# rogerhh/gaussian-splatting-lm

Measured on AMD Instinct MI355X. Metric: CG matvecs/sec + raster Mpix/s, 1M Gaussians @1080p, 1/2/4/8 GPU, higher is better.
Workload: dtype f32; 1 GPU; LM CG iteration, 1000000 Gaussians SH3, 1x1920x1080 view(s) per GPU (BASELINE configs[2]; configs[3] at 8 GPUs); P=1000000, sh_degree=3, width=1920, height=1080, views_total=1, parallelism=views sharded x1, exchange=none, sh_rest_projected=True

## Files before the change

### gaussian-splatting-lm_amd/csrc/api.hip

```cpp
#include <cstring>
#include <string>
#include <vector>
#include "gslm_kernels.hpp"

namespace gslm {

static thread_local std::string g_last_error;
void set_error(const std::string& msg) { g_last_error = msg; }

thread_local DebugSync g_debug;

int launch_failed(hipError_t e, const char* file, int line) {
  const char* base = std::strrchr(file, '/');
  set_error(std::string(g_debug.on ? "kernel failed (debug mode: stream synchronised after the launch at " : "kernel launch (") +
            (base ? base + 1 : file) + ":" + std::to_string(line) + "): " + hipGetErrorString(e));
  return GSLM_ERR_HIP;
}

namespace {

struct Carver {
  char* base;
  size_t off = 0;
  template <typename T>
// ... 1031 lines not shown
}

size_t gslm_active_union_bytes(int64_t P) { return active_work_layout(P, nullptr, nullptr, nullptr, nullptr); }

int gslm_active_union(const gslm_view_ws* ws, int32_t nviews, int64_t P, void* work, size_t work_bytes, int32_t* ids_dev,
                      uint32_t* hrow_dev, uint32_t* aflags_dev, int64_t* count_dev, void* stream) {
  if (!ws || nviews < 1 || P < 0 || P > MAX_P || !work || !count_dev || !hrow_dev || (P > 0 && (!ids_dev || !aflags_dev))) {
    set_error("active_union: NULL argument, nviews below 1 or P out of range");
    return GSLM_ERR_INVALID;
  }
  for (int b = 0; b < nviews; ++b)
    if (ws[b].num_rendered < 0 || (ws[b].num_rendered > 0 && P > 0 && (!ws[b].geom || !ws[b].scratch))) {
      set_error("active_union: negative num_rendered or a NULL workspace of a view that rendered");
      return GSLM_ERR_INVALID;
    }
  if (work_bytes < gslm_active_union_bytes(P)) {
    set_error("active_union: work area below gslm_active_union_bytes(P)");
    return GSLM_ERR_CAPACITY;
  }
  for (int b = 0; b < nviews; ++b)
    if (ws[b].num_rendered > 0 && ws[b].scratch_bytes < gslm_scratch_bytes(P, ws[b].num_rendered)) {
      set_error("active_union: scratch workspace too small");
      return GSLM_ERR_CAPACITY;
    }
  std::vector<GeomBufs> gbs(nviews);
  std::vector<ScratchBufs> sbs(nviews);
  std::vector<int64_t> nr(nviews);
  for (int b = 0; b < nviews; ++b) {
    nr[b] = ws[b].num_rendered;
    if (nr[b] == 0) continue;
    geom_layout(P, const_cast<void*>(ws[b].geom), &gbs[b]);
    scratch_layout(P, nr[b], const_cast<void*>(ws[b].scratch), &sbs[b]);
  }
  uint32_t *flags, *tmp, *total;
  active_work_layout(P, work, &flags, &tmp, &total);
  return launch_active_union(gbs.data(), sbs.data(), nr.data(), nviews, P, flags, tmp, total, ids_dev, hrow_dev,
                             aflags_dev, count_dev, (hipStream_t)stream);
}

int gslm_inspect_rowmap(const void* geom, int64_t P, int64_t N, const void* scratch, size_t scratch_bytes,
                        uint32_t* goff, uint32_t* hscan, void* stream) {
  if (P < 0 || N < 0 || !geom || !scratch) { set_error("inspect_rowmap: NULL workspace or negative size"); return GSLM_ERR_INVALID; }
  if (scratch_bytes < gslm_scratch_bytes(P, N)) { set_error("inspect_rowmap: scratch workspace too small"); return GSLM_ERR_CAPACITY; }
  GeomBufs gb;
  ScratchBufs sb;
  geom_layout(P, const_cast<void*>(geom), &gb);
  scratch_layout(P, N, const_cast<void*>(scratch), &sb);
  hipStream_t s = (hipStream_t)stream;
  if (goff && P > 0) GSLM_HIP_CHECK(hipMemcpyAsync(goff, gb.goff, (size_t)P * 4, hipMemcpyDeviceToDevice, s));
  if (hscan) GSLM_HIP_CHECK(hipMemcpyAsync(hscan, sb.hscan, (size_t)(N + 1) * 4, hipMemcpyDeviceToDevice, s));
  return GSLM_OK;
}

int gslm_active_pack(const float* src, float* dst, const int32_t* active_ids, int64_t n_active, int64_t P,
                     const int32_t* widths, int32_t ngroups, int64_t tail_n, void* stream) {
  return launch_active_pack(true, src, dst, active_ids, n_active, P, widths, ngroups, tail_n, (hipStream_t)stream);
}

int gslm_active_unpack(const float* src, float* dst, const int32_t* active_ids, int64_t n_active, int64_t P,
                       const int32_t* widths, int32_t ngroups, int64_t tail_n, void* stream) {
  return launch_active_pack(false, src, dst, active_ids, n_active, P, widths, ngroups, tail_n, (hipStream_t)stream);
}

int gslm_sh_rest_project(const gslm_view* view, const gslm_gaussians* gi, int32_t mode, const float* in,
                         int64_t in_stride, float* out, int64_t out_stride, void* stream) {
  ViewK v;
  GaussK g;
  int st;
  if (!view || !gi) { set_error("sh_rest_project: NULL view / gaussians"); return GSLM_ERR_INVALID; }
  if ((st = make_view(view, gi->max_coeffs, &v))) return st;
  if ((st = make_gauss(gi, &v, &g, false))) return st;
  if (mode != 0 && mode != 1) { set_error("sh_rest_project: mode must be 0 (expand) or 1 (project)"); return GSLM_ERR_INVALID; }
  if (g.P > 0 && g.M > 1 && (!in || !out || !g.means3D)) { set_error("sh_rest_project: NULL buffer"); return GSLM_ERR_INVALID; }
  const int64_t full = 3 * (int64_t)(g.M - 1);
  if ((mode == 0 && (in_stride < 3 || out_stride < full)) || (mode == 1 && (in_stride < full || out_stride < 3))) {
    set_error("sh_rest_project: strides too small for [P,3] / [P,M-1,3] rows");
    return GSLM_ERR_INVALID;
  }
  return launch_sh_rest_project(v, g, mode, in, in_stride, out, out_stride, (hipStream_t)stream);
}

static int rest_views(const char* who, const gslm_view* views, int32_t nviews, const gslm_gaussians* gi, ViewK* vk,
                      GaussK* g) {
  if (!views || !gi || nviews < 1 || nviews > GSLM_MAX_REST_VIEWS) {
    set_error(std::string(who) + ": NULL views / gaussians or nviews outside 1..GSLM_MAX_REST_VIEWS");
    return GSLM_ERR_INVALID;
  }
  int st;
  for (int b = 0; b < nviews; ++b) {
    if ((st = make_view(&views[b], gi->max_coeffs, &vk[b]))) return st;
    if (vk[b].D != vk[0].D) {
      set_error(std::string(who) + ": the views must share one SH degree");
      return GSLM_ERR_INVALID;
    }
  }
  if ((st = make_gauss(gi, &vk[0], g, false))) return st;
  if (g->P > 0 && !g->means3D) {
    set_error(std::string(who) + ": NULL means3D");
    return GSLM_ERR_INVALID;
  }
  return GSLM_OK;
}

int gslm_rest_basis(const gslm_view* views, int32_t nviews, const gslm_gaussians* gi, float* R_out, void* stream) {
  ViewK vk[GSLM_MAX_REST_VIEWS];
  GaussK g;
// ... 247 lines not shown
```

### gaussian-splatting-lm_amd/csrc/forward.hip

```cpp
#include "gslm_internal.hpp"
#include "gslm_kernels.hpp"

namespace gslm {

template <bool RAW, bool STAGE>
__global__ __launch_bounds__(256) void k_preprocess(ViewK v, GaussK g, float4* __restrict__ rec,
                                                     uint32_t* __restrict__ depth_key,
                                                     uint32_t* __restrict__ tiles, uint2* __restrict__ rect,
                                                     uint32_t* __restrict__ clampw, int* __restrict__ radii_out,
                                                     int lead) {
  extern __shared__ __attribute__((aligned(16))) float s_sh[];
  const int64_t i = (int64_t)blockIdx.x * blockDim.x + threadIdx.x;
  if (STAGE) {
    const int64_t i0 = (int64_t)blockIdx.x * blockDim.x;
    const int64_t nv = min((int64_t)blockDim.x, g.P - i0);
    const int64_t total = nv * g.rest_stride;
    const float* rows = g.rest - lead + i0 * g.rest_stride;
    const float4* src4 = reinterpret_cast<const float4*>(rows);
    float4* dst4 = reinterpret_cast<float4*>(s_sh);
    for (int64_t e = threadIdx.x; e < total / 4; e += blockDim.x) dst4[e] = src4[e];
    for (int64_t e = (total / 4) * 4 + threadIdx.x; e < total; e += blockDim.x) s_sh[e] = rows[e];
    __syncthreads();
    g.rest = s_sh + lead;
    g.rest_base = i0;
  }
  if (i >= g.P) return;
  tiles[i] = 0u;
  depth_key[i] = 0xFFFFFFFFu;
  if (radii_out) radii_out[i] = 0;
  PreOut o;
  o.depth = 0.f;
  const bool vis = preprocess_one<RAW>(v, g, i, o);
  if (o.depth > 0.2f) depth_key[i] = __float_as_uint(o.depth);
  if (!vis) return;

  const float4 r0 = make_float4(o.x, o.y, o.conic[0], o.conic[1]);
  const float4 r1 = make_float4(o.conic[2], o.opac, o.rgb[0], o.rgb[1]);
  const float4 r2 = make_float4(o.rgb[2], 1.0f / o.depth, __uint_as_float(o.clamped), o.tq);
  rec[RECS * i + 0] = r0;
  rec[RECS * i + 1] = r1;
  rec[RECS * i + 2] = r2;
  tiles[i] = (uint32_t)((o.rmax_x - o.rmin_x) * (o.rmax_y - o.rmin_y));
  const uint2 rc = make_uint2((uint32_t)o.rmin_x | ((uint32_t)o.rmin_y << 16), (uint32_t)o.rmax_x | ((uint32_t)o.rmax_y << 16));
  rect[i] = rc;
  rec[RECS * i + 3] = make_float4(__uint_as_float(rc.x), __uint_as_float(rc.y), 0.f, 0.f);
  clampw[i] = o.clamped;
  if (radii_out) radii_out[i] = o.radius;
}

__device__ __forceinline__ void glds16(const float4* src, float4* lds_dst) {
  __builtin_amdgcn_global_load_lds((const __attribute__((address_space(1))) void*)src,
                                   (__attribute__((address_space(3))) void*)lds_dst, 16, 0, 0);
}

// ... 389 lines not shown
}

__global__ __launch_bounds__(256) void k_tile_neff(ViewK v, const uint32_t* __restrict__ n_contrib,
                                                    uint32_t* __restrict__ neff) {
  const int tile = blockIdx.x, tile_x = tile % v.gx, tile_y = tile / v.gx;
  int px, py;
  tile_pixel(tile_x, tile_y, threadIdx.x, px, py);
  int wm = (px < v.W && py < v.H) ? (int)n_contrib[(int64_t)py * v.W + px] : 0;
#pragma unroll
  for (int o = 32; o >= 1; o >>= 1) wm = max(wm, __shfl_xor(wm, o));
  if ((threadIdx.x & 63) == 0) neff[4 * tile + (threadIdx.x >> 6)] = (uint32_t)wm;
}

__global__ __launch_bounds__(256) void k_tile_cost(const uint2* __restrict__ ranges,
                                                    const uint32_t* __restrict__ point_list,
                                                    const uint32_t* __restrict__ neff, uint32_t* __restrict__ cost) {
  __shared__ uint32_t s_c[4][4];
  const int tile = blockIdx.x, tid = threadIdx.x, w = tid >> 6;
  const uint2 r = ranges[tile];
  const uint32_t len = r.y - r.x;
  uint32_t wm[4];
#pragma unroll
  for (int q = 0; q < 4; ++q) wm[q] = min(neff[4 * tile + q], len);
  const int n_eff = (int)max(max(wm[0], wm[1]), max(wm[2], wm[3]));
  uint32_t tot[4] = {0u, 0u, 0u, 0u}, vjp = 0u;
  for (int base = 0; base < n_eff; base += 256) {
    const int pos = n_eff - 1 - (base + tid);
    uint32_t m = 0u;
    if (pos >= 0) {
      const uint32_t e = point_list[r.x + pos];
      m = pl_mask(e) & (((uint32_t)pos < wm[0] ? 1u : 0u) | ((uint32_t)pos < wm[1] ? 2u : 0u) |
                        ((uint32_t)pos < wm[2] ? 4u : 0u) | ((uint32_t)pos < wm[3] ? 8u : 0u));
    }
#pragma unroll
    for (int q = 0; q < 4; ++q) {
      const uint32_t c = (uint32_t)__popcll(__ballot((m >> q) & 1u));
      if ((tid & 63) == 0) s_c[w][q] = c;
    }
    __syncthreads();
    uint32_t b0 = 0u, b1 = 0u;
#pragma unroll
    for (int q = 0; q < 4; ++q) {
      const uint32_t c0 = s_c[0][q] + s_c[1][q], c1 = s_c[2][q] + s_c[3][q];
      tot[q] += c0 + c1;
      b0 = max(b0, c0);
      b1 = max(b1, c1);
    }
    vjp += b0 + b1;
    __syncthreads();
  }
  if (tid == 0) cost[tile] = max(max(tot[0], tot[1]), max(tot[2], tot[3])) + vjp;
}

__device__ __forceinline__ uint32_t eff_mask(uint32_t e, uint32_t pos, const uint32_t* wm4) {
  const uint32_t wb = (pos < wm4[0] ? 1u : 0u) | (pos < wm4[1] ? 2u : 0u) | (pos < wm4[2] ? 4u : 0u) |
                      (pos < wm4[3] ? 8u : 0u);
  return pl_mask(e) & wb;
}

__global__ __launch_bounds__(256) void k_row_flags(int64_t N, int gx, const uint32_t* __restrict__ keys,
                                                    const uint32_t* __restrict__ point_list,
                                                    const uint2* __restrict__ ranges, const uint32_t* __restrict__ neff,
                                                    const uint32_t* __restrict__ goff, const uint2* __restrict__ rect,
                                                    uint32_t* __restrict__ slots, uint32_t* __restrict__ flags) {
  const int64_t k = (int64_t)blockIdx.x * blockDim.x + threadIdx.x;
  if (k >= N) return;
  const uint32_t t = keys[k];
  const uint32_t e = point_list[k];
  const uint32_t g = pl_id(e);
  const uint32_t o = row_slot(goff[g], rect[g], (int)(t % (uint32_t)gx), (int)(t / (uint32_t)gx));
  slots[k] = o;
  flags[o] = eff_mask(e, (uint32_t)k - ranges[t].x, neff + 4 * (size_t)t) ? 1u : 0u;
}

__global__ __launch_bounds__(256) void k_row_final(int64_t N, const uint32_t* __restrict__ hscan,
                                                    uint32_t* __restrict__ slots) {
  const int64_t k = (int64_t)blockIdx.x * blockDim.x + threadIdx.x;
  if (k < N) slots[k] = hscan[slots[k]];
}

int launch_lm_rowmap(const ViewK& v, const GeomBufs& gb, const BinBufs& bb, const ImgBufs& ib, const ScratchBufs& sb,
                     int64_t N, hipStream_t s) {
  const int ntiles = v.gx * v.gy;
  if (N <= 0 || ntiles == 0) {
    GSLM_HIP_CHECK(hipMemsetAsync(sb.hscan, 0, sizeof(uint32_t), s));
    return GSLM_OK;
  }
  const unsigned nb = (unsigned)((N + 255) / 256);
  hipLaunchKernelGGL(k_tile_neff, dim3(ntiles), dim3(TILE_PIX), 0, s, v, ib.n_contrib, bb.tile_neff);
  if (N + 1 >= ntiles) {
    hipLaunchKernelGGL(k_tile_cost, dim3(ntiles), dim3(256), 0, s, bb.ranges, bb.point_list, bb.tile_neff, sb.hscan);
    if (int st = launch_tile_order(ntiles, bb.ranges, bb.tile_order, sb.hscan, s)) return st;
  }
  hipLaunchKernelGGL(k_row_flags, dim3(nb), dim3(256), 0, s, N, v.gx, bb.keys_sorted, bb.point_list, bb.ranges,
                     bb.tile_neff, gb.goff, gb.rect, bb.slots, sb.hscan);
  GSLM_LAUNCH_CHECK();
  const int st = exclusive_scan_u32(sb.hscan, nullptr, sb.hscan, N, sb.scan_tmp, sb.hscan + N, s);
  if (st) return st;
  hipLaunchKernelGGL(k_row_final, dim3(nb), dim3(256), 0, s, N, sb.hscan, bb.slots);
  GSLM_LAUNCH_CHECK();
  return GSLM_OK;
}

__device__ __forceinline__ uint32_t owns_head_row(int64_t i, const uint32_t* __restrict__ tiles,
                                                  const uint32_t* __restrict__ goff,
                                                  const uint32_t* __restrict__ hscan) {
  const uint32_t n = tiles[i];
  if (n == 0) return 0u;
  const uint32_t o = goff[i];
  return hscan[o + n] > hscan[o] ? 1u : 0u;
}

__global__ __launch_bounds__(256) void k_active_flags(int64_t P, const uint32_t* __restrict__ tiles,
                                                       const uint32_t* __restrict__ goff,
                                                       const uint32_t* __restrict__ hscan, uint32_t* __restrict__ flags) {
  const int64_t i = (int64_t)blockIdx.x * blockDim.x + threadIdx.x;
  if (i < P) flags[i] = owns_head_row(i, tiles, goff, hscan);
}

__global__ __launch_bounds__(256) void k_active_scatter(int64_t P, int64_t N, const uint32_t* __restrict__ tiles,
                                                         const uint32_t* __restrict__ goff,
                                                         const uint32_t* __restrict__ hscan,
                                                         const uint32_t* __restrict__ pos,
                                                         const uint32_t* __restrict__ total, int32_t* __restrict__ ids,
                                                         uint32_t* __restrict__ hrow, int64_t* __restrict__ count) {
  const int64_t i = (int64_t)blockIdx.x * blockDim.x + threadIdx.x;
  if (i == 0) {
    *count = (int64_t)*total;
    hrow[*total] = hscan[N];
  }
  if (i < P && owns_head_row(i, tiles, goff, hscan)) {
    ids[pos[i]] = (int32_t)i;
    hrow[pos[i]] = hscan[goff[i]];
  }
}

int launch_active_list(int64_t P, int64_t N, const GeomBufs& gb, const ScratchBufs& sb, uint32_t* flags,
                       uint32_t* scan_tmp, uint32_t* total, int32_t* ids, uint32_t* hrow, int64_t* count,
                       hipStream_t s) {
  if (P <= 0) {
    GSLM_HIP_CHECK(hipMemsetAsync(count, 0, sizeof(int64_t), s));
    GSLM_HIP_CHECK(hipMemsetAsync(hrow, 0, sizeof(uint32_t), s));
// ... 342 lines not shown
```

### gaussian-splatting-lm_amd/gslm/_lib.py

```python
import ctypes
import math
import os

import torch

_HERE = os.path.dirname(os.path.abspath(__file__))
_DEFAULT_LIB = os.path.join(os.path.dirname(_HERE), "build", "libgslm.so")
LIB_PATH = os.environ.get("GSLM_LIB", _DEFAULT_LIB)

GSLM_OK = 0
GSLM_ERR_INVALID = -1
GSLM_ERR_HIP = -2
GSLM_ERR_CAPACITY = -3
GSLM_MAX_REST_VIEWS = 8


class GslmView(ctypes.Structure):
    _fields_ = [
        ("image_height", ctypes.c_int32), ("image_width", ctypes.c_int32),
        ("tanfovx", ctypes.c_double), ("tanfovy", ctypes.c_double), ("scale_modifier", ctypes.c_double),
        ("viewmatrix", ctypes.c_float * 16), ("projmatrix", ctypes.c_float * 16),
        ("campos", ctypes.c_float * 3), ("bg", ctypes.c_float * 3),
        ("sh_degree", ctypes.c_int32), ("prefiltered", ctypes.c_int32),
        ("antialiasing", ctypes.c_int32), ("debug", ctypes.c_int32),
# ... 257 lines not shown
    "gslm_xpby_dev": (ctypes.c_int, [ctypes.c_int64, ctypes.c_void_p, ctypes.c_void_p, ctypes.c_void_p,
                                     ctypes.c_void_p, ctypes.c_void_p]),
    "gslm_damp_add": (ctypes.c_int, [ctypes.c_int64, ctypes.c_void_p, ctypes.POINTER(ctypes.c_int64),
                                     ctypes.POINTER(ctypes.c_double), ctypes.c_int32, ctypes.c_void_p,
                                     ctypes.c_void_p]),
    "gslm_comm_id_bytes": (ctypes.c_int32, []),
    "gslm_comm_unique_id": (ctypes.c_int, [ctypes.c_void_p]),
    "gslm_comm_init": (ctypes.c_int, [ctypes.c_void_p, ctypes.c_int32, ctypes.c_int32,
                                      ctypes.POINTER(ctypes.c_void_p)]),
    "gslm_comm_destroy": (ctypes.c_int, [ctypes.c_void_p]),
    "gslm_allreduce_sum_f32": (ctypes.c_int, [ctypes.c_void_p, ctypes.c_void_p, ctypes.c_int64, ctypes.c_void_p]),
    "gslm_allreduce_sum_f64": (ctypes.c_int, [ctypes.c_void_p, ctypes.c_void_p, ctypes.c_int64, ctypes.c_void_p]),
    "gslm_alltoall": (ctypes.c_int, [ctypes.c_void_p, ctypes.c_void_p, ctypes.c_void_p, ctypes.c_int64,
                                     ctypes.c_void_p]),
    "gslm_allgather": (ctypes.c_int, [ctypes.c_void_p, ctypes.c_void_p, ctypes.c_void_p, ctypes.c_int64,
                                      ctypes.c_void_p]),
    "gslm_residual_scratch_bytes": (ctypes.c_size_t, [ctypes.c_int32, ctypes.c_int32]),
    "gslm_lm_residual": (ctypes.c_int, [ctypes.c_int32, ctypes.c_int32, ctypes.c_void_p, ctypes.c_void_p,
                                        ctypes.c_void_p, ctypes.c_void_p, ctypes.c_void_p, ctypes.c_void_p,
                                        ctypes.c_void_p, ctypes.c_size_t, ctypes.c_void_p, ctypes.c_int32,
                                        ctypes.c_void_p]),
    "gslm_exposure_scratch_bytes": (ctypes.c_size_t, [ctypes.c_int32, ctypes.c_int32]),
    "gslm_lm_residual_exposure": (ctypes.c_int, [ctypes.c_int32, ctypes.c_int32, ctypes.c_void_p, ctypes.c_void_p,
                                                 ctypes.c_void_p, ctypes.c_void_p, ctypes.c_void_p, ctypes.c_void_p,
                                                 ctypes.c_void_p, ctypes.c_void_p, ctypes.c_void_p, ctypes.c_size_t,
                                                 ctypes.c_void_p, ctypes.c_int32, ctypes.c_void_p]),
    "gslm_ssim_state_bytes": (ctypes.c_size_t, [ctypes.c_int32, ctypes.c_int32]),
    "gslm_ssim_residual": (ctypes.c_int, [ctypes.c_int32, ctypes.c_int32, ctypes.c_void_p, ctypes.c_void_p,
                                          ctypes.c_void_p, ctypes.c_float, ctypes.c_void_p, ctypes.c_size_t,
                                          ctypes.c_void_p, ctypes.c_void_p, ctypes.c_void_p, ctypes.c_void_p,
                                          ctypes.c_int32, ctypes.c_void_p]),
    "gslm_ssim_normal": (ctypes.c_int, [ctypes.c_int32, ctypes.c_int32, ctypes.c_void_p, ctypes.c_void_p,
                                        ctypes.c_void_p, ctypes.c_void_p, ctypes.c_void_p]),
    "gslm_ssim_mean_state_bytes": (ctypes.c_size_t, [ctypes.c_int32, ctypes.c_int32, ctypes.c_int32]),
    "gslm_ssim_mean": (ctypes.c_int, [ctypes.c_int32, ctypes.c_int32, ctypes.c_int32, ctypes.c_void_p, ctypes.c_void_p,
                                      ctypes.c_void_p, ctypes.c_size_t, ctypes.c_void_p, ctypes.c_void_p]),
    "gslm_ssim_mean_backward": (ctypes.c_int, [ctypes.c_int32, ctypes.c_int32, ctypes.c_int32, ctypes.c_void_p,
                                               ctypes.c_void_p, ctypes.c_void_p, ctypes.c_void_p, ctypes.c_void_p,
                                               ctypes.c_void_p]),
    "gslm_knn_scratch_bytes": (ctypes.c_size_t, [ctypes.c_int64]),
    "gslm_knn3_mean_dist": (ctypes.c_int, [ctypes.c_int64, ctypes.c_void_p, ctypes.c_void_p, ctypes.c_void_p,
                                           ctypes.c_size_t, ctypes.c_void_p]),
    "gslm_adam_step": (ctypes.c_int, [ctypes.POINTER(GslmAdamGroup), ctypes.c_int32, ctypes.c_double, ctypes.c_double,
                                      ctypes.c_double, ctypes.c_void_p, ctypes.c_int64, ctypes.c_int32,
                                      ctypes.c_void_p]),
    "gslm_densify_stats": (ctypes.c_int, [ctypes.c_int64, ctypes.c_void_p, ctypes.c_int64, ctypes.c_void_p,
                                          ctypes.c_void_p, ctypes.c_void_p, ctypes.c_void_p, ctypes.c_void_p]),
    "gslm_inspect": (ctypes.c_int, [ctypes.c_void_p, ctypes.c_int64, ctypes.c_void_p, ctypes.c_int64, ctypes.c_int32,
                                    ctypes.c_int32, ctypes.c_void_p, ctypes.c_void_p, ctypes.c_void_p,
                                    ctypes.c_void_p, ctypes.c_void_p, ctypes.c_void_p, ctypes.c_void_p,
                                    ctypes.c_void_p]),
    "gslm_inspect_rowmap": (ctypes.c_int, [ctypes.c_void_p, ctypes.c_int64, ctypes.c_int64, ctypes.c_void_p,
                                           ctypes.c_size_t, ctypes.c_void_p, ctypes.c_void_p, ctypes.c_void_p]),
    "gslm_selftest": (ctypes.c_int, [ctypes.c_int32, ctypes.c_void_p, ctypes.c_void_p, ctypes.c_void_p]),
    "gslm_selftest_scan": (ctypes.c_int, [ctypes.c_void_p, ctypes.c_void_p, ctypes.c_int64, ctypes.c_int32,
                                          ctypes.c_void_p, ctypes.c_size_t, ctypes.c_void_p, ctypes.c_void_p]),
    "gslm_selftest_scan_dual": (ctypes.c_int, [ctypes.c_void_p, ctypes.c_void_p, ctypes.c_void_p, ctypes.c_void_p,
                                               ctypes.c_void_p, ctypes.c_int64, ctypes.c_int32, ctypes.c_void_p,
                                               ctypes.c_size_t, ctypes.c_void_p, ctypes.c_void_p, ctypes.c_void_p]),
    "gslm_selftest_sort_hist_bytes": (ctypes.c_size_t, [ctypes.c_int64, ctypes.c_int32]),
    "gslm_selftest_sort": (ctypes.c_int, [ctypes.c_void_p, ctypes.c_void_p, ctypes.c_void_p, ctypes.c_void_p,
                                          ctypes.c_void_p, ctypes.c_void_p, ctypes.c_int64, ctypes.c_int32,
                                          ctypes.c_int32, ctypes.c_int32, ctypes.c_void_p, ctypes.c_void_p,
                                          ctypes.c_void_p, ctypes.c_size_t, ctypes.POINTER(ctypes.c_int32),
                                          ctypes.c_void_p]),
    "gslm_selftest_ranges": (ctypes.c_int, [ctypes.c_void_p, ctypes.c_int64, ctypes.c_int32, ctypes.c_void_p,
                                            ctypes.c_void_p, ctypes.c_void_p, ctypes.c_void_p]),
    "gslm_selftest_tile_order": (ctypes.c_int, [ctypes.c_void_p, ctypes.c_void_p, ctypes.c_int32, ctypes.c_int32,
                                                ctypes.c_void_p, ctypes.c_void_p]),
    "gslm_last_error": (ctypes.c_char_p, []),
    "gslm_abi_version": (ctypes.c_int, []),
}


ABI_VERSION = 9


class GslmError(RuntimeError):
    pass


def _load():
    if not os.path.exists(LIB_PATH):
        raise ImportError(f"libgslm.so not found at {LIB_PATH}: build it with "
                          f"`python -c 'import __graft_entry__ as g; g.build()'` (hipcc, gfx950)")
    lib = ctypes.CDLL(LIB_PATH)
    ab_mode = os.environ.get("GSLM_ABI_ANY") == "1" and "GSLM_LIB" in os.environ and LIB_PATH != _DEFAULT_LIB
    for name, (restype, argtypes) in EXPORTS.items():
        if ab_mode and not hasattr(lib, name):
            continue
        fn = getattr(lib, name)
        fn.restype = restype
        fn.argtypes = argtypes
    if lib.gslm_abi_version() != ABI_VERSION:
        if not (os.environ.get("GSLM_ABI_ANY") == "1" and "GSLM_LIB" in os.environ and LIB_PATH != _DEFAULT_LIB):
            raise ImportError(f"{LIB_PATH} has C ABI version {lib.gslm_abi_version()}, these bindings need "
                              f"{ABI_VERSION}: rebuild it")
        import warnings
        warnings.warn(f"gslm: GSLM_ABI_ANY=1 loads {LIB_PATH} (ABI {lib.gslm_abi_version()}) into ABI "
                      f"{ABI_VERSION} bindings: A/B timing only, struct layouts are not checked", RuntimeWarning)
    return lib


lib = _load()


# ... 113 lines not shown
```

### gaussian-splatting-lm_amd/gslm/lm.py

```python
import copy
import ctypes
import math
import os

import torch

from gslm import _lib
from gslm._lib import check, lib
from gslm.params import GROUPS, ParamLayout, raw_gaussians

STAGE_ALL = 7
STAGE_OVERWRITE = 8
MV_TAIL_CLEAN = 1
MV_SH_REST_PROJECTED = 2
MV_LEAN = 4
MV_EXPOSURE = 8

DEFAULT_DAMP = {"xyz": 5e2, "features_dc": 5e-2, "features_rest": 5e-2, "scaling": 5e-2, "rotation": 5e-2,
                "opacity": 5e-2, "exposure": 1e1}


class ViewRaster:

    def __init__(self, view, device):
        self.view = view
        self.H, self.W = view.image_height, view.image_width
        self.device = device
        self.N = 0
        self.geom = self.binning = self.image = self.scratch = None
        self._active = None
        self._params = None
        self.tail_clean = False
        self.epoch = 0

    @property
    def tail_clean(self):
        return self._tail_clean

    @tail_clean.setter
    def tail_clean(self, value):
        self._tail_clean = bool(value)
        if not value:
            self._active = None
            self._params = None

    def active_list(self, P, stream):
        if not self.tail_clean or self.N is None:
            raise RuntimeError("active_list: no current LM row map (run a product or rhs() on this geometry first)")
        if self._active is None:
            dev = self.device
            ids = torch.empty(max(P, 1), dtype=torch.int32, device=dev)
            rows = torch.empty(P + 1, dtype=torch.int32, device=dev)
            count = torch.zeros(1, dtype=torch.int64, device=dev)
            work = _lib.u8(lib.gslm_active_list_bytes(P), dev)
            check(lib.gslm_active_list(self.geom.data_ptr(), P, self.N, self.scratch.data_ptr(), self.scratch.numel(),
                                       work.data_ptr(), work.numel(), ids.data_ptr(), rows.data_ptr(),
                                       count.data_ptr(), stream), "gslm_active_list")
            n = int(count.item())
            self._active = (ids[:n], n)
            self.active_rows = rows[:n + 1]
        return self._active

    def active_params(self, model, P, stream):
        ids, na = self.active_list(P, stream)
        leaves = (model._xyz, model._scaling, model._rotation, model._opacity)
        key = tuple((t.data_ptr(), t._version) for t in leaves)
        if self._params is None or self._params[0] != key:
            dev = self.device
            block = _lib.u8(lib.gslm_active_params_bytes(na), dev)
            pos = torch.empty(max(P, 1), dtype=torch.int32, device=dev)
            g = raw_gaussians(model)
            check(lib.gslm_active_params(ctypes.byref(g), self.geom.data_ptr(), P, ids.data_ptr() if na else None, na,
                                         block.data_ptr(), block.numel(), pos.data_ptr(), stream), "gslm_active_params")
            self._params = (key, block, pos)
        return self._params[1], self._params[2]

    def forward(self, g, stream, want_invdepth=True):
        P = g.P
        dev = self.device
        self.tail_clean = False
        self.epoch += 1
        if self.geom is None or self.geom.numel() < lib.gslm_geom_bytes(P):
            self.geom = _lib.u8(lib.gslm_geom_bytes(P), dev)
            self.image = _lib.u8(lib.gslm_image_bytes(self.H, self.W), dev)
            self.color = torch.empty(3, self.H, self.W, dtype=torch.float32, device=dev)
            self.invdepth = torch.empty(1, self.H, self.W, dtype=torch.float32, device=dev)
            self.radii = torch.empty(P, dtype=torch.int32, device=dev)
        check(lib.gslm_preprocess(ctypes.byref(self.view), ctypes.byref(g), self.geom.data_ptr(), self.geom.numel(),
                                  self.radii.data_ptr(), stream), "gslm_preprocess")
        n = ctypes.c_int64(0)
        check(lib.gslm_num_rendered(self.geom.data_ptr(), P, ctypes.byref(n), stream), "gslm_num_rendered")
        self.N = int(n.value)
        need = lib.gslm_binning_bytes(self.N, self.H, self.W)
        if self.binning is None or self.binning.numel() < need:
            self.binning = _lib.u8(int(need * 1.25) + 4096, dev)
        check(lib.gslm_rasterize(ctypes.byref(self.view), P, self.geom.data_ptr(), self.binning.data_ptr(),
                                 self.binning.numel(), self.N, self.image.data_ptr(), self.image.numel(),
                                 self.color.data_ptr(), self.invdepth.data_ptr() if want_invdepth else None, stream),
              "gslm_rasterize")
        need = lib.gslm_scratch_bytes(P, self.N)
        if self.scratch is None or self.scratch.numel() < need:
            self.scratch = _lib.u8(int(need * 1.25) + 4096, dev)
        return self.color


    def forward_dev(self, g, stream, want_invdepth=True, n_out=None):
        if self.binning is None or self.geom is None or self.geom.numel() < lib.gslm_geom_bytes(g.P):
            raise RuntimeError("forward_dev: the workspaces of an earlier forward() at this P are required")
        P = g.P
        self.tail_clean = False
        self.epoch += 1
        self.N = None
        check(lib.gslm_preprocess(ctypes.byref(self.view), ctypes.byref(g), self.geom.data_ptr(), self.geom.numel(),
                                  self.radii.data_ptr(), stream), "gslm_preprocess")
# ... 20 lines not shown
        self.bg = bg
        self.mask_xyz = bool(mask_xyz)
        self.train_exposure = bool(train_exposure)
        if self.train_exposure:
            self._init_exposure(model, cams, device)
        P = model._xyz.shape[0]
        K = 1 + model._features_rest.shape[1]
        if sh_projection == "auto":
            sh_projection = len(cams) == 1 and K > 1 and model.active_sh_degree > 0
        if sh_projection and len(cams) != 1:
            raise ValueError("sh_projection is a single-view mode (the Krylov space of one view's J)")
        self.full_layout = ParamLayout(P, K, model._exposure.shape[0])
        self.layout = ParamLayout(P, K, model._exposure.shape[0], rest_projected=bool(sh_projection))
        self.mv_flags = MV_SH_REST_PROJECTED if self.layout.rest_projected else 0
        self.damp = DEFAULT_DAMP if damp is None else damp
        self._bounds, self._damps = self.layout.group_damp_arrays(self.damp)
        self.gts = [c.original_image.to(device) for c in cams] if gts is None else gts
        self.masks = [c.alpha_mask.to(device) for c in cams] if alpha_masks is None else alpha_masks
        self.views = [ViewRaster(_lib.view_from_camera(c, bg, model.active_sh_degree), device) for c in cams]
        self.stream = _lib.stream_handle(device)
        self.dot_scratch = torch.empty(max(lib.gslm_dot_scratch_bytes(max(P, self.layout.numel)) // 8, 3 * 1024) + 8,
                                       dtype=torch.float64, device=device)
        self.weights = [None] * len(cams)
        self.residuals = [None] * len(cams)
        self.seeds = [None] * len(cams)
        self.ssim_state = [None] * len(cams)
        self._jv = [None] * len(cams)
        self._u = [None] * len(cams)
        self.res_scratch = torch.empty(lib.gslm_residual_scratch_bytes(1, 1) // 8, dtype=torch.float64,
                                       device=device)

    def _init_exposure(self, model, cams, device):
        if self.ssim or not self.mask_xyz:
            raise ValueError("train_exposure runs on the LM rows with the plain residual (mask_xyz=True, ssim=False)")
        if getattr(model, "pretrained_exposures", None) is not None:
            raise ValueError("train_exposure: the model renders with pretrained exposures, which are not parameters")
        missing = [c.image_name for c in cams if c.image_name not in model.exposure_mapping]
        if missing:
            raise ValueError(f"train_exposure: no row of model._exposure for {missing} (model.exposure_mapping)")
        X = model._exposure
        if X.dtype != torch.float32 or not X.is_contiguous() or X.shape[1:] != (3, 4):
            raise ValueError("train_exposure: model._exposure must be contiguous float32 [n, 3, 4]")
        self.exp_idx = [int(model.exposure_mapping[c.image_name]) for c in cams]
        self._exp_rhs = torch.zeros(X.numel(), dtype=torch.float32, device=device)
        self._exp_u = [None] * len(cams)
        self._exp_scratch = torch.empty(lib.gslm_exposure_scratch_bytes(1, 1) // 8, dtype=torch.float64,
                                        device=device)
        seen = set()
        self._exp_first = [not (i in seen or seen.add(i)) for i in self.exp_idx]
        rest = sorted(set(range(X.shape[0])) - seen)
        self._exp_rest = torch.tensor(rest, dtype=torch.long, device=device) if rest else None

    def evaluate(self):
        g = raw_gaussians(self.model)
        loss = torch.zeros((), dtype=torch.float64, device=self.device)
        if self.train_exposure:
            self._exp_rhs.zero_()
        for b, vr in enumerate(self.views):
            R = vr.forward(g, self.stream, want_invdepth=False)
            if self.residuals[b] is None or self.residuals[b].shape != R.shape:
                self.residuals[b] = torch.empty_like(R)
                self.weights[b] = torch.empty_like(R)
                self.seeds[b] = torch.empty_like(R)
                if self.train_exposure:
                    self._exp_u[b] = torch.empty_like(R)
            m = self.masks[b]
            gt = self.gts[b]
            if m is not None:
                m = m.to(torch.float32).contiguous()
                if m.numel() != vr.H * vr.W:
                    raise ValueError("alpha mask must be [1, H, W]")
            if gt.shape != R.shape or gt.dtype != torch.float32:
                raise ValueError(f"ground truth must be float32 {tuple(R.shape)}, got {gt.dtype} {tuple(gt.shape)}")
            gt = gt.contiguous()
            if self.ssim:
                if self.ssim_state[b] is None:
                    self.ssim_state[b] = _lib.u8(lib.gslm_ssim_state_bytes(vr.H, vr.W), self.device)
                    self._jv[b] = torch.empty_like(R)
                    self._u[b] = torch.empty_like(R)
                st = self.ssim_state[b]
                check(lib.gslm_ssim_residual(vr.H, vr.W, R.data_ptr(), gt.data_ptr(),
                                             None if m is None else m.data_ptr(), self.lambda_dssim, st.data_ptr(),
                                             st.numel(), None, None, self.seeds[b].data_ptr(), loss.data_ptr(),
                                             int(b > 0), self.stream), "gslm_ssim_residual")
                continue
            if self.train_exposure:
                check(lib.gslm_lm_residual_exposure(
                    vr.H, vr.W, R.data_ptr(), gt.data_ptr(), None if m is None else m.data_ptr(),
                    self.model._exposure.data_ptr() + 48 * self.exp_idx[b], self.residuals[b].data_ptr(),
                    self.weights[b].data_ptr(), self.seeds[b].data_ptr(),
                    self._exp_rhs.data_ptr() + 48 * self.exp_idx[b], self._exp_scratch.data_ptr(),
                    self._exp_scratch.numel() * 8, loss.data_ptr(), int(b > 0), self.stream),
                    "gslm_lm_residual_exposure")
                continue
            check(lib.gslm_lm_residual(vr.H, vr.W, R.data_ptr(), gt.data_ptr(), None if m is None else m.data_ptr(),
                                       self.residuals[b].data_ptr(), self.weights[b].data_ptr(),
                                       self.seeds[b].data_ptr(), self.res_scratch.data_ptr(),
                                       self.res_scratch.numel() * 8, loss.data_ptr(), int(b > 0), self.stream),
                  "gslm_lm_residual")
        self.loss = loss
        return loss

    def num_rendered(self):
        return [v.N for v in self.views]

    def rhs(self, out, fused=True):
# ... 956 lines not shown
        prob.jt_residual(r, rm, s)
        s -= Dx(x)
        p = s.clone()
        gamma = float((s.double() * s.double()).sum())
        for _ in range(restart_iter):
            q = [t.clone() for t in prob.jv_residual(p, rm, jv)]
            delta = dot2(q, q) + ddot(p, p)
            if delta < 1e-20:
                if verbose:
                    print("Early termination: delta is too small.")
                stop = True
                break
            alpha = gamma / delta
            x += alpha * p
            r = [rr - alpha * qq for rr, qq in zip(r, q)]
            prob.jt_residual(r, rm, s)
            s -= Dx(x)
            gamma_prev, gamma = gamma, float((s.double() * s.double()).sum())
            p = s + (gamma / gamma_prev) * p
            prob.jv_residual(x, rm, jv)
            cur = [bb - q for bb, q in zip(b, jv)]
            res = dot2(cur, cur) + ddot(x, x)
            history.append(res)
            if verbose:
                print(f"[Iter {iter_total + 1}] res: {res:.2e}")
            if res > last_res:
                stop = True
                break
            last_res = res
            if callback is not None:
                callback(x, s, iter_total + 1)
            if gamma < max(tol * math.sqrt(gamma_prev), atol):
                stop = True
                break
            iter_total += 1
            if iter_total >= max_iter:
                stop = True
                break
    return x, {"iters": iter_total, "residuals": history}


def loss_set_group():
    if "GSLM_LOSS_SETS" in os.environ:
        raise ValueError("GSLM_LOSS_SETS is no longer read: set GSLM_LOSS_SET_GROUP=k (k sets per blend pass, 1..8; "
                         "1 = per set, the default; 8 = all sets in one pass)")
    raw = os.environ.get("GSLM_LOSS_SET_GROUP", "1")
    try:
        k = int(raw)
    except ValueError:
        k = 0
    if not 1 <= k <= 8:
        raise ValueError(f"GSLM_LOSS_SET_GROUP={raw!r}: sets per blend pass must be an integer in 1..8")
    return k


class LossEvaluator:

    def __init__(self, model, cams, bg, device="cuda", batch=8, gts=None, alpha_masks=None, reduce=None, streams=3,
                 device_count=False, train_exposure=False, fused_exposure=False):
        self.model = model
        self.train_exposure = bool(train_exposure)
        self.fused_exposure = bool(fused_exposure)
        if self.fused_exposure and not self.train_exposure:
            raise ValueError("fused_exposure=True is an option of train_exposure=True")
        if self.fused_exposure and device_count:
            raise ValueError("fused_exposure=True: the device-count blend has no exposure form (device_count=False)")
        if self.train_exposure:
            if getattr(model, "pretrained_exposures", None) is not None:
                raise ValueError("train_exposure: the model renders with pretrained exposures, which are not parameters")
            missing = [c.image_name for c in cams if c.image_name not in model.exposure_mapping]
            if missing:
                raise ValueError(f"train_exposure: no row of model._exposure for {missing} (model.exposure_mapping)")
            self.exp_idx = [int(model.exposure_mapping[c.image_name]) for c in cams]
        if self.train_exposure and not self.fused_exposure:
            self._exp_scratch = torch.empty(lib.gslm_exposure_scratch_bytes(1, 1) // 8, dtype=torch.float64,
                                            device=device)
            self._exp_raster = {}
        self.device_count = device_count
        self.device = device
        self.reduce = reduce
        self.gts = [c.original_image.to(device) for c in cams] if gts is None else gts
        ms = [c.alpha_mask for c in cams] if alpha_masks is None else alpha_masks
        self.masks = [None if m is None else m.to(device=device, dtype=torch.float32).contiguous() for m in ms]
        self.views = [_lib.view_from_camera(c, bg, model.active_sh_degree) for c in cams]
        for vw, gt, m in zip(self.views, self.gts, self.masks):
            H, W = vw.image_height, vw.image_width
            if gt.shape != (3, H, W) or gt.dtype != torch.float32:
                raise ValueError(f"ground truth must be float32 (3, {H}, {W}), got {gt.dtype} {tuple(gt.shape)}")
            if m is not None and m.numel() != H * W:
                raise ValueError("alpha mask must be [1, H, W]")
        self.batch = max(1, min(int(batch), len(cams) or 1))
        nstr = max(1, min(int(streams), self.batch))
        self.streams = [torch.cuda.Stream(device) for _ in range(nstr)] if nstr > 1 else [None]
        self.slots = [dict(geom=None, binning=None) for _ in range(self.batch)]
        nb = max([lib.gslm_loss_scratch_bytes(v.image_height, v.image_width) for v in self.views] + [8])
        self.loss_scratch = [torch.empty(nb // 8 + 1, dtype=torch.float64, device=device) for _ in self.streams]
        self.num_rendered = [0] * len(cams)
        self._order_key, self._orders = None, [None] * len(cams)
        self._pos = [None] * len(cams)
        self.uslots = [[dict(geoms=[], ugeom=None) for _ in range(self.batch)] for _ in range(2)]
        self.ubins = [None] * self.batch
        self.sets_scratch = [None] * self.batch
        self.loss_sets = loss_set_group()
        self.union_counts = []

    def _slot(self, k, P):
# ... 491 lines not shown
```

### include/gslm.h

```cpp
#ifndef GSLM_H
#define GSLM_H

#include <stddef.h>
#include <stdint.h>

#ifdef __cplusplus
extern "C" {
#endif

#define GSLM_OK 0
#define GSLM_ERR_INVALID (-1)
#define GSLM_ERR_HIP (-2)
#define GSLM_ERR_CAPACITY (-3)

#define GSLM_ABI_VERSION 9

typedef struct gslm_view {
  int32_t image_height;
  int32_t image_width;
  double tanfovx;
  double tanfovy;
  double scale_modifier;
  float viewmatrix[16];
  float projmatrix[16];
// ... 278 lines not shown
int32_t gslm_comm_id_bytes(void);
int gslm_comm_unique_id(void* id_out);
int gslm_comm_init(const void* id, int32_t nranks, int32_t rank, void** comm_out);
int gslm_comm_destroy(void* comm);
int gslm_allreduce_sum_f32(void* comm, float* buf, int64_t n, void* stream);
int gslm_allreduce_sum_f64(void* comm, double* buf, int64_t n, void* stream);
int gslm_alltoall(void* comm, const void* send, void* recv, int64_t bytes_per_rank, void* stream);
int gslm_allgather(void* comm, const void* send, void* recv, int64_t bytes_per_rank, void* stream);

size_t gslm_residual_scratch_bytes(int32_t H, int32_t W);
int gslm_lm_residual(int32_t H, int32_t W, const float* color, const float* gt, const float* alpha_mask,
                     float* residual, float* weight, float* seed, void* scratch, size_t scratch_bytes,
                     double* loss_dev, int32_t accumulate, void* stream);

size_t gslm_ssim_state_bytes(int32_t H, int32_t W);
int gslm_ssim_residual(int32_t H, int32_t W, const float* color, const float* gt, const float* alpha_mask,
                       float lambda_dssim, void* state, size_t state_bytes, float* r1, float* r2, float* seed,
                       double* loss_dev, int32_t accumulate, void* stream);
int gslm_ssim_normal(int32_t H, int32_t W, const float* gt, void* state, const float* jv, float* u, void* stream);

size_t gslm_ssim_mean_state_bytes(int32_t C, int32_t H, int32_t W);
int gslm_ssim_mean(int32_t C, int32_t H, int32_t W, const float* img, const float* gt, void* state,
                   size_t state_bytes, float* ssim_out, void* stream);
int gslm_ssim_mean_backward(int32_t C, int32_t H, int32_t W, const float* img, const float* gt, const void* state,
                            const float* grad_out, float* grad_img, void* stream);

size_t gslm_knn_scratch_bytes(int64_t n);
int gslm_knn3_mean_dist(int64_t n, const float* xyz, float* out, void* scratch, size_t scratch_bytes, void* stream);

#define GSLM_ADAM_MAX_GROUPS 8
typedef struct gslm_adam_group {
  float* param;
  const float* grad;
  float* exp_avg;
  float* exp_avg_sq;
  int64_t n;
  int32_t floats_per_gaussian;
  int32_t _pad;
  double lr;
  int64_t step;
} gslm_adam_group;
int gslm_adam_step(const gslm_adam_group* groups, int32_t ngroups, double beta1, double beta2, double eps,
                   const uint8_t* visible, int64_t num_gaussians, int32_t sparse, void* stream);
int gslm_densify_stats(int64_t P, const float* means2D_grad, int64_t grad_stride, const int32_t* radii,
                       float* max_radii2D, float* xyz_gradient_accum, float* denom, void* stream);

int gslm_inspect(const void* geom, int64_t P, const void* binning, int64_t num_rendered, int32_t H, int32_t W,
                 const void* image, uint32_t* point_list, uint32_t* ranges, uint32_t* tiles_touched,
                 float* final_T, uint32_t* n_contrib, float* records, void* stream);

int gslm_inspect_rowmap(const void* geom, int64_t P, int64_t num_rendered, const void* scratch, size_t scratch_bytes,
                        uint32_t* goff, uint32_t* hscan, void* stream);

int gslm_selftest(int32_t which, const float* in, float* out, void* stream);
int gslm_selftest_scan(const uint32_t* in, uint32_t* out, int64_t n, int32_t force_top, void* tmp, size_t tmp_bytes,
                       uint32_t* total, void* stream);
int gslm_selftest_scan_dual(const uint32_t* in, const uint32_t* idx, const uint32_t* in_b, uint32_t* out_a,
                            uint32_t* out_b, int64_t n, int32_t force_top, void* tmp, size_t tmp_bytes,
                            uint32_t* total_a, uint32_t* total_b, void* stream);
size_t gslm_selftest_sort_hist_bytes(int64_t n, int32_t payload);
int gslm_selftest_sort(uint32_t* k0, uint32_t* v0, uint32_t* k1, uint32_t* v1, uint32_t* p0, uint32_t* p1, int64_t n,
                       int32_t end_bit, int32_t iota_values, int32_t key_range, const uint32_t* last_gather,
                       const uint32_t* n_dev, void* hist, size_t hist_bytes, int32_t* result_in_alt, void* stream);
int gslm_selftest_ranges(const uint32_t* keys, int64_t n, int32_t ntiles, const uint32_t* n_dev, uint32_t* n_out,
                         uint32_t* ranges, void* stream);
int gslm_selftest_tile_order(const uint32_t* ranges, const uint32_t* cost, int32_t ntiles, int32_t form,
                             uint32_t* order, void* stream);

const char* gslm_last_error(void);
int gslm_abi_version(void);

#ifdef __cplusplus
}
#endif
#endif
```

Measured before the change: 1785 view-matvec/s (one (J^T J + D) application per 1080p view, 1M Gaussians).

## Prune point-list quadrant mask bits for Gaussians dead in each quadrant

Adds a kernel that runs after the forward render and evaluates each listed Gaussian against every pixel of each 64-pixel tile quadrant. It clears the quadrant bit in the point-list word when no pixel in that quadrant receives a contribution (past its last contributor, positive power, or alpha below 1/255). Later row-map, cost and matvec passes that read the masks then skip that quadrant. The goal is to cut wasted Jacobian work in the CG matvecs, at the cost of an extra per-tile pass with atomics on the point list. It is on by default behind an env switch, and an inspect entry point is added for debugging.

```diff
diff --git a/gaussian-splatting-lm_amd/csrc/api.hip b/gaussian-splatting-lm_amd/csrc/api.hip
--- a/gaussian-splatting-lm_amd/csrc/api.hip
+++ b/gaussian-splatting-lm_amd/csrc/api.hip
@@ -1107,6 +1107,18 @@
   return GSLM_OK;
 }
 
+int gslm_inspect_list(const void* binning, size_t binning_bytes, int64_t N, int32_t H, int32_t W, uint32_t* words,
+                      uint32_t* slots, void* stream) {
+  if (N < 0 || H <= 0 || W <= 0 || !binning) { set_error("inspect_list: NULL binning, negative count or empty image"); return GSLM_ERR_INVALID; }
+  if (binning_bytes < gslm_binning_bytes(N, H, W)) { set_error("inspect_list: binning workspace too small"); return GSLM_ERR_CAPACITY; }
+  BinBufs bb;
+  bin_layout(N, ((W + TILE_X - 1) / TILE_X) * ((H + TILE_Y - 1) / TILE_Y), const_cast<void*>(binning), &bb);
+  hipStream_t s = (hipStream_t)stream;
+  if (words && N > 0) GSLM_HIP_CHECK(hipMemcpyAsync(words, bb.point_list, (size_t)N * 4, hipMemcpyDeviceToDevice, s));
+  if (slots && N > 0) GSLM_HIP_CHECK(hipMemcpyAsync(slots, bb.slots, (size_t)N * 4, hipMemcpyDeviceToDevice, s));
+  return GSLM_OK;
+}
+
 int gslm_active_pack(const float* src, float* dst, const int32_t* active_ids, int64_t n_active, int64_t P,
                      const int32_t* widths, int32_t ngroups, int64_t tail_n, void* stream) {
   return launch_active_pack(true, src, dst, active_ids, n_active, P, widths, ngroups, tail_n, (hipStream_t)stream);
diff --git a/gaussian-splatting-lm_amd/csrc/forward.hip b/gaussian-splatting-lm_amd/csrc/forward.hip
--- a/gaussian-splatting-lm_amd/csrc/forward.hip
+++ b/gaussian-splatting-lm_amd/csrc/forward.hip
@@ -1,5 +1,6 @@
 #include "gslm_internal.hpp"
 #include "gslm_kernels.hpp"
+#include "gslm_tile.hpp"
 
 namespace gslm {
 
@@ -495,6 +496,65 @@
   if (tid == 0) cost[tile] = max(max(tot[0], tot[1]), max(tot[2], tot[3])) + vjp;
 }
 
+static bool live_masks_on() {
+  const char* e = getenv("GSLM_LIVE_MASKS");
+  return !(e && std::string(e) == "0");
+}
+
+__global__ __launch_bounds__(256) void k_quad_live(ViewK v, const uint2* __restrict__ ranges,
+                                                    const uint32_t* __restrict__ tile_order,
+                                                    const uint32_t* __restrict__ neff,
+                                                    const float4* __restrict__ rec,
+                                                    const uint32_t* __restrict__ n_contrib, uint32_t* point_list) {
+  __shared__ float4 s_a[4][64];
+  __shared__ float2 s_b[4][64];
+  const int tile = (int)tile_order[blockIdx.x];
+  const int tile_x = tile % v.gx, tile_y = tile / v.gx;
+  const int tid = threadIdx.x, q = tid >> 6, lane = tid & 63;
+  int px, py;
+  tile_pixel(tile_x, tile_y, tid, px, py);
+  const bool inside = px < v.W && py < v.H;
+  const uint32_t my_last = inside ? n_contrib[(int64_t)py * v.W + px] : 0u;
+  const uint2 range = ranges[tile];
+  const int wm = __builtin_amdgcn_readfirstlane((int)min(neff[4 * tile + q], range.y - range.x));
+  const float pxf = (float)px, pyf = (float)py;
+  uint32_t* pl = point_list + range.x;
+  float4* sa = s_a[q];
+  float2* sb = s_b[q];
+  for (int base = 0; base < wm; base += 64) {
+    const int k = base + lane;
+    bool hit = false;
+    if (k < wm) {
+      const uint32_t e = __hip_atomic_load(pl + k, __ATOMIC_RELAXED, __HIP_MEMORY_SCOPE_AGENT);
+      if ((pl_mask(e) >> q) & 1u) {
+        hit = true;
+        const uint32_t g = pl_id(e);
+        const float4 r0 = rec[RECS * (size_t)g + 0], r1 = rec[RECS * (size_t)g + 1];
+        sa[lane] = r0;
+        sb[lane] = make_float2(r1.x, r1.y);
+      }
+    }
+    uint64_t hb = __ballot(hit);
+    const int rel = (int)my_last - base;
+    uint64_t live = 0ull;
+    wave_lds_sync();
+    while (hb) {
+      const int j = (int)__builtin_ctzll(hb);
+      hb = clear_bit(hb, j);
+      const float4 a = sa[j];
+      const float2 b = sb[j];
+      const float dx = a.x - pxf, dy = a.y - pyf;
+      const float power = gpower(a.z, a.w, b.x, dx, dy);
+      const float G = gexp(power);
+      const float alpha = fminf(0.99f, b.y * G);
+      const bool c_last = j < rel, c_pow = !(power > 0.0f), c_alpha = alpha >= 1.0f / 255.0f;
+      if (__builtin_amdgcn_ballot_w64(c_last && c_pow && c_alpha)) live |= 1ull << j;
+    }
+    if (hit && !((live >> lane) & 1ull)) atomicAnd(pl + k, ~(1u << (ID_BITS + q)));
+    wave_lds_sync();
+  }
+}
+
 __device__ __forceinline__ uint32_t eff_mask(uint32_t e, uint32_t pos, const uint32_t* wm4) {
   const uint32_t wb = (pos < wm4[0] ? 1u : 0u) | (pos < wm4[1] ? 2u : 0u) | (pos < wm4[2] ? 4u : 0u) |
                       (pos < wm4[3] ? 8u : 0u);
@@ -531,6 +591,9 @@
   }
   const unsigned nb = (unsigned)((N + 255) / 256);
   hipLaunchKernelGGL(k_tile_neff, dim3(ntiles), dim3(TILE_PIX), 0, s, v, ib.n_contrib, bb.tile_neff);
+  if (live_masks_on())
+    hipLaunchKernelGGL(k_quad_live, dim3(ntiles), dim3(TILE_PIX), 0, s, v, bb.ranges, bb.tile_order, bb.tile_neff,
+                       gb.rec, ib.n_contrib, bb.point_list);
   if (N + 1 >= ntiles) {
     hipLaunchKernelGGL(k_tile_cost, dim3(ntiles), dim3(256), 0, s, bb.ranges, bb.point_list, bb.tile_neff, sb.hscan);
     if (int st = launch_tile_order(ntiles, bb.ranges, bb.tile_order, sb.hscan, s)) return st;
diff --git a/gaussian-splatting-lm_amd/gslm/_lib.py b/gaussian-splatting-lm_amd/gslm/_lib.py
--- a/gaussian-splatting-lm_amd/gslm/_lib.py
+++ b/gaussian-splatting-lm_amd/gslm/_lib.py
@@ -333,6 +333,8 @@
                                     ctypes.c_void_p]),
     "gslm_inspect_rowmap": (ctypes.c_int, [ctypes.c_void_p, ctypes.c_int64, ctypes.c_int64, ctypes.c_void_p,
                                            ctypes.c_size_t, ctypes.c_void_p, ctypes.c_void_p, ctypes.c_void_p]),
+    "gslm_inspect_list": (ctypes.c_int, [ctypes.c_void_p, ctypes.c_size_t, ctypes.c_int64, ctypes.c_int32,
+                                         ctypes.c_int32, ctypes.c_void_p, ctypes.c_void_p, ctypes.c_void_p]),
     "gslm_selftest": (ctypes.c_int, [ctypes.c_int32, ctypes.c_void_p, ctypes.c_void_p, ctypes.c_void_p]),
     "gslm_selftest_scan": (ctypes.c_int, [ctypes.c_void_p, ctypes.c_void_p, ctypes.c_int64, ctypes.c_int32,
                                           ctypes.c_void_p, ctypes.c_size_t, ctypes.c_void_p, ctypes.c_void_p]),
diff --git a/gaussian-splatting-lm_amd/gslm/lm.py b/gaussian-splatting-lm_amd/gslm/lm.py
--- a/gaussian-splatting-lm_amd/gslm/lm.py
+++ b/gaussian-splatting-lm_amd/gslm/lm.py
@@ -60,6 +60,14 @@
             self._active = (ids[:n], n)
             self.active_rows = rows[:n + 1]
         return self._active
+
+    def list_words(self, stream):
+        n = max(self.N, 1)
+        words = torch.zeros(n, dtype=torch.int32, device=self.device)
+        slots = torch.zeros(n, dtype=torch.int32, device=self.device)
+        check(lib.gslm_inspect_list(self.binning.data_ptr(), self.binning.numel(), self.N, self.H, self.W,
+                                    words.data_ptr(), slots.data_ptr(), stream), "gslm_inspect_list")
+        return words[:self.N], slots[:self.N]
 
     def active_params(self, model, P, stream):
         ids, na = self.active_list(P, stream)
@@ -186,6 +194,7 @@
         self._exp_rest = torch.tensor(rest, dtype=torch.long, device=device) if rest else None
 
     def evaluate(self):
+        live_masks()
         g = raw_gaussians(self.model)
         loss = torch.zeros((), dtype=torch.float64, device=self.device)
         if self.train_exposure:
@@ -1248,6 +1257,13 @@
     if not 1 <= k <= 8:
         raise ValueError(f"GSLM_LOSS_SET_GROUP={raw!r}: sets per blend pass must be an integer in 1..8")
     return k
+
+
+def live_masks():
+    raw = os.environ.get("GSLM_LIVE_MASKS", "1")
+    if raw not in ("0", "1"):
+        raise ValueError(f"GSLM_LIVE_MASKS={raw!r}: 1 (refine the quadrant masks, the default) or 0")
+    return raw == "1"
 
 
 class LossEvaluator:
diff --git a/include/gslm.h b/include/gslm.h
--- a/include/gslm.h
+++ b/include/gslm.h
@@ -354,6 +354,9 @@
 int gslm_inspect_rowmap(const void* geom, int64_t P, int64_t num_rendered, const void* scratch, size_t scratch_bytes,
                         uint32_t* goff, uint32_t* hscan, void* stream);
 
+int gslm_inspect_list(const void* binning, size_t binning_bytes, int64_t num_rendered, int32_t H, int32_t W,
+                      uint32_t* words, uint32_t* slots, void* stream);
+
 int gslm_selftest(int32_t which, const float* in, float* out, void* stream);
 int gslm_selftest_scan(const uint32_t* in, uint32_t* out, int64_t n, int32_t force_top, void* tmp, size_t tmp_bytes,
                        uint32_t* total, void* stream);
```

Result: faster. 1872 view-matvec/s (one (J^T J + D) application per 1080p view, 1M Gaussians) (median of 6 runs) (+4.8%).
